# Ruyi-Zha/r2_gaussian

Hardware: AMD Instinct MI355X
Metric: rasterized X-ray views/sec (fwd+bwd) at 300k Gaussians, 512^2 cone-beam detector (higher is better)
Workload: dtype f32

## Files before the change

### r2_gaussian_amd/csrc/raster_geom.hip

```cpp
#include "r2_math.hpp"
#include "raster_state.hpp"

R2_TS_DEFINE(geom)

#ifndef M_PI
#define M_PI 3.14159265358979323846
#endif

namespace r2 {

__device__ __forceinline__ float ndc2pix(float v, int S) { return (float)((((double)v + 1.0) * (double)S - 1.0) * 0.5); }

struct Cov2D {
    float tx, ty, tz;
    float xmul, ymul;
    M3 J, W, M, cov;
};

__device__ __forceinline__ void cov2d_common(float3 mean, float fx, float fy, float tan_fovx, float tan_fovy,
                                             const float *cov3D, const float *__restrict__ view, int mode, Cov2D &c)
{
    float3 t = xform4x3(mean, view);
    if (mode == 0) {
        const float limx = 1.3f, limy = 1.3f;
        t.x = fminf(limx, fmaxf(-limx, t.x));
        t.y = fminf(limx, fmaxf(-limx, t.y));
        c.xmul = (t.x < -limx || t.x > limx) ? 0.f : 1.f;
        c.ymul = (t.y < -limy || t.y > limy) ? 0.f : 1.f;
        c.J = m3(fx, 0.0f, 0.0f, 0.0f, fy, 0.0f, 0.0f, 0.0f, 1.0f);
    } else {
        const float limx = 1.3f * tan_fovx, limy = 1.3f * tan_fovy;
        const float txtz = t.x / t.z, tytz = t.y / t.z;
        t.x = fminf(limx, fmaxf(-limx, txtz)) * t.z;
        t.y = fminf(limy, fmaxf(-limy, tytz)) * t.z;
        c.xmul = (txtz < -limx || txtz > limx) ? 0.f : 1.f;
        c.ymul = (tytz < -limy || tytz > limy) ? 0.f : 1.f;
        const float l = sqrtf(t.x * t.x + t.y * t.y + t.z * t.z);
        c.J = m3(fx / t.z, 0.0f, -(fx * t.x) / (t.z * t.z), 0.0f, fy / t.z, -(fy * t.y) / (t.z * t.z), t.x / l, t.y / l,
                 t.z / l);
    }
    c.tx = t.x; c.ty = t.y; c.tz = t.z;
    c.W = m3(view[0], view[4], view[8], view[1], view[5], view[9], view[2], view[6], view[10]);
    c.M = mul(c.W, c.J);
    const M3 Vrk = m3(cov3D[0], cov3D[1], cov3D[2], cov3D[1], cov3D[3], cov3D[4], cov3D[2], cov3D[4], cov3D[5]);
    c.cov = mul(mul(tr(c.M), tr(Vrk)), c.M);
}

__device__ __forceinline__ float mu_of(float circ, float diamond)
{
    const double q = 2 * M_PI * (double)circ / (double)diamond;
    float mu = 0.0f;
    if ((float)q > 0.0f) mu = (float)sqrt(q);
    return mu;
}

__device__ __forceinline__ void raster_preprocess_one(
    int idx , int src , const float *__restrict__ means3D, const float *__restrict__ scales, float scale_modifier,
    const float *__restrict__ rotations, const float *__restrict__ opacities, const float *__restrict__ cov3D_precomp,
    const float *__restrict__ view, const float *__restrict__ proj, int W, int H, float tan_fovx, float tan_fovy,
    float focal_x, float focal_y, int mode, int gx, int gy,
    int *__restrict__ radii, float4 *__restrict__ rec, uint32_t *__restrict__ depth_key,
    float *__restrict__ cov3Ds, uint32_t *__restrict__ tiles_touched, float2 *__restrict__ op_mu,
    uint32_t *__restrict__ thin_flag, const DepthReg &reg, uint32_t &key_out, uint2 &bt_out, uint32_t &rect_out)
{
    key_out = DEPTH_CULLED_KEY;
    radii[idx] = 0;
    tiles_touched[idx] = 0;
    depth_key[idx] = 0xFFFFFFFFu;

    const float3 p = make_float3(means3D[3 * src], means3D[3 * src + 1], means3D[3 * src + 2]);
    const float3 p_view = xform4x3(p, view);
    if (p_view.z <= 0.2f) return;
    const float4 p_hom = xform4x4(p, proj);
    const float p_w = 1.0f / (p_hom.w + 0.0000001f);
    const float projx = p_hom.x * p_w, projy = p_hom.y * p_w;

    float cov3D[6];
    if (cov3D_precomp != nullptr) {
#pragma unroll
        for (int k = 0; k < 6; ++k) cov3D[k] = cov3D_precomp[6 * src + k];
    } else {
        const float4 q = reinterpret_cast<const float4 *>(rotations)[src];
        cov3d_from_scale_rot(scales[3 * src], scales[3 * src + 1], scales[3 * src + 2], scale_modifier, q, cov3D);
        if (cov3Ds != nullptr)
#pragma unroll
            for (int k = 0; k < 6; ++k) cov3Ds[6 * idx + k] = cov3D[k];
    }

    Cov2D c;
    cov2d_common(p, focal_x, focal_y, tan_fovx, tan_fovy, cov3D, view, mode, c);
    const float a = c.cov.m[0][0], b = c.cov.m[0][1], cc = c.cov.m[0][2];
    const float d = c.cov.m[1][1], e = c.cov.m[1][2], f = c.cov.m[2][2];
    const float diamond = a * d - b * b;
    const float circ = a * d * f + 2 * b * cc * e - a * e * e - f * b * b - d * cc * cc;
    const float mu = mu_of(circ, diamond);

    const float det = (a * d - b * b);
    if (det == 0.0f) return;
    const float det_inv = 1.f / det;
    const float conA = d * det_inv, conB = -b * det_inv, conC = a * det_inv;

    const float mid = 0.5f * (a + d);
    const float lambda1 = mid + sqrtf(fmaxf(0.1f, mid * mid - det));
    const float lambda2 = mid - sqrtf(fmaxf(0.1f, mid * mid - det));
    const float my_radius = ceilf(3.f * sqrtf(fmaxf(lambda1, lambda2)));
    const float px = ndc2pix(projx, W), py = ndc2pix(projy, H);
    int x0, y0, x1, y1;
    tile_rect(px, py, (int)my_radius, gx, gy, x0, y0, x1, y1);
    if ((uint32_t)(x1 - x0) * (uint32_t)(y1 - y0) == 0) return;

    depth_key[idx] = __float_as_uint(p_view.z);
    radii[idx] = (int)my_radius;
    tiles_touched[idx] = (uint32_t)(y1 - y0) * (uint32_t)(x1 - x0);
    key_out = __float_as_uint(p_view.z);
    bt_out = depth_register_key(reg, key_out, (uint32_t)(y1 - y0) * (uint32_t)(x1 - x0));
    rect_out = depth_rect_pack(x0, y0, x1 - x0, y1 - y0);
    const float op = opacities[src];
    const float opmu = op * mu;
    const float L = opmu > 0.0f ? log2f(opmu) : -INFINITY;
    float hx = INFINITY, hy = INFINITY;
    {
        const double qmax = 2.0 * (double)LN2 * ((double)L - (double)LOG2_ALPHA_MIN_2D) + 1e-3;
        const double A = conA, B = conB, C = conC;
        const double det2 = A * C - B * B, trc = A + C;
        if (!(qmax > 0.0)) {
            hx = hy = -INFINITY;
        } else if (det2 > 0.0 && A > 0.0 && C > 0.0 && trc * trc <= 1.0e4 * det2) {
            const double ex = sqrt(qmax * C / det2) * 1.004 + 0.05, ey = sqrt(qmax * A / det2) * 1.004 + 0.05;
            if (ex < 1.0e30 && ey < 1.0e30) { hx = (float)ex; hy = (float)ey; }
        }
    }
    rec[2 * idx] = make_float4(px, py, (-0.5f * LOG2E) * conA, (-LOG2E) * conB);
    rec[2 * idx + 1] = make_float4((-0.5f * LOG2E) * conC, L, hx, hy);
    op_mu[idx] = make_float2(op, mu);
    if (thin_flag && hx > 0.f && item_tier((-0.5f * LOG2E) * conA, (-LOG2E) * conB, (-0.5f * LOG2E) * conC, L, hx, hy) != 0) *thin_flag = 1u;
}

__global__ void __launch_bounds__(256) raster_preprocess_kernel(
    int P, int V, const float *__restrict__ means3D, const float *__restrict__ scales, float scale_modifier,
    const float *__restrict__ rotations, const float *__restrict__ opacities, const float *__restrict__ cov3D_precomp,
    const float *__restrict__ views, const float *__restrict__ projs, int W, int H, float tan_fovx, float tan_fovy,
    float focal_x, float focal_y, int mode, int gx, int gy,
    int *__restrict__ radii, float4 *__restrict__ rec, uint32_t *__restrict__ depth_key,
    float *__restrict__ cov3Ds, uint32_t *__restrict__ tiles_touched, float2 *__restrict__ op_mu,
    uint32_t *__restrict__ thin_flag, DepthReg reg)
{
    const int idx = blockIdx.x * 256 + threadIdx.x;
    R2_TS_AT(geom, 0);
    uint32_t key = DEPTH_CULLED_KEY;
    uint2 bt = make_uint2(0u, 0u);
    uint32_t rect = 0u, thin = 0u;
    if (idx < P * V) {
        const int v = V == 1 ? 0 : idx / P;
        raster_preprocess_one(idx, idx - v * P, means3D, scales, scale_modifier, rotations, opacities, cov3D_precomp, views + 16 * v,
                              projs + 16 * v, W, H, tan_fovx, tan_fovy, focal_x, focal_y, mode, gx, gy, radii, rec, depth_key, cov3Ds,
                              tiles_touched, op_mu, &thin, reg, key, bt, rect);
    }
    if (thin_flag != nullptr) {
        const uint32_t nthin = (uint32_t)__popcll(__ballot(thin != 0u));
        if (nthin != 0u && (threadIdx.x & 63) == 0) atomicAdd(thin_flag, nthin);
    }
    R2_TS_AT(geom, 1);
    depth_register_end(reg, (uint32_t)idx, key, bt, rect);
    R2_TS_AT(geom, 2);
}

template <bool SL , bool SHARE, bool MV>
__global__ void __launch_bounds__(TF_THREADS_MAX, SHARE ? 8 : 4) raster_preprocess_tf_kernel(
    int P , int V ,
    uint32_t per_wg, const TFSlabs slabs, const float *__restrict__ means3D, const float *__restrict__ scales, float scale_modifier,
    const float *__restrict__ rotations, const float *__restrict__ opacities, const float *__restrict__ cov3D_precomp,
    const float *__restrict__ view, const float *__restrict__ proj, int W, int H, float tan_fovx, float tan_fovy,
    float focal_x, float focal_y, int mode, int gx, int gy,
    int *__restrict__ radii, float4 *__restrict__ rec, uint32_t *__restrict__ depth_key,
    float *__restrict__ cov3Ds, uint32_t *__restrict__ tiles_touched, float2 *__restrict__ op_mu,
    uint32_t *__restrict__ first, uint32_t *__restrict__ rects, uint32_t *__restrict__ wgoff, uint32_t *__restrict__ wgmm,
    TFCounters *__restrict__ ctr)
{
    extern __shared__ uint32_t tf_hist[];
    constexpr int MAXW = (int)(TF_THREADS_MAX / 64), NI = (int)TF_PER_THREAD_MAX;
    __shared__ uint32_t s_wn[NI][MAXW], s_wv[MAXW], s_kmx[MAXW], s_nkmn[MAXW], s_thin, s_base;
    const int tid = threadIdx.x, lane = tid & 63, wave = tid >> 6;
    const uint32_t NT = blockDim.x;
    const int nw = (int)(NT >> 6);
    const uint32_t nsl = SL ? slabs.n : 1u;
    const uint32_t T = (uint32_t)(gx * gy * (MV ? V : 1)) * nsl;
    const uint32_t PV = (uint32_t)P * (uint32_t)(MV ? V : 1);
    const uint32_t g0 = blockIdx.x * per_wg, g1 = min(g0 + per_wg, PV);
    R2_TS_AT(geom, 0);
    for (uint32_t t = tid; t < T; t += NT) tf_hist[t] = 0u;
    if (tid == 0) s_thin = 0u;
    uint32_t key[NI], rect[NI], thin = 0u;
    const DepthReg noreg{};
#pragma unroll
    for (int it = 0; it < NI; ++it) {
        key[it] = DEPTH_CULLED_KEY; rect[it] = 0u;
        const uint32_t idx = g0 + (uint32_t)it * NT + (uint32_t)tid;
        uint2 bt = make_uint2(0u, 0u);
        if ((it == 0 || NT * (uint32_t)it < per_wg) && idx < g1) {
            const uint32_t v = MV ? idx / (uint32_t)P : 0u;
            raster_preprocess_one((int)idx, (int)(idx - v * (uint32_t)P), means3D, scales, scale_modifier, rotations, opacities,
                                  cov3D_precomp, view + 16u * v, proj + 16u * v, W, H, tan_fovx, tan_fovy, focal_x, focal_y, mode, gx, gy,
                                  radii, rec, depth_key, cov3Ds, tiles_touched, op_mu, &thin, noreg, key[it], bt, rect[it]);
            if (MV && key[it] != DEPTH_CULLED_KEY) rect[it] += (v * (uint32_t)gy) << 8;
        }
    }
    R2_TS_AT(geom, 10);
    __syncthreads();
    uint32_t n[NI], incl[NI], nvis = 0u, kmx = 0u, nkmn = 0u;
#pragma unroll
    for (int it = 0; it < NI; ++it) {
        const bool vis = key[it] != DEPTH_CULLED_KEY;
        n[it] = vis ? depth_rect_count(rect[it]) : 0u;
        if (vis) {
            const uint32_t x0 = rect[it] & 0xFFu, y0 = (rect[it] >> 8) & 0xFFu, w = ((rect[it] >> 16) & 0xFFu) + 1u, h = (rect[it] >> 24) + 1u;
            const uint32_t sl = SL ? tf_slab_of(key[it], slabs) : 0u;
            for (uint32_t r = 0; r < h; ++r) {
                const uint32_t row = ((y0 + r) * (uint32_t)gx + x0) * nsl + sl;
                for (uint32_t c = 0; c < w; ++c) atomicAdd(&tf_hist[row + c * nsl], 1u);
            }
            rects[g0 + (uint32_t)it * NT + (uint32_t)tid] = rect[it];
            kmx = max(kmx, key[it]);
            nkmn = max(nkmn, ~key[it]);
        }
        incl[it] = n[it];
#pragma unroll
        for (int d = 1; d < 64; d <<= 1) {
            const uint32_t up = __shfl_up(incl[it], d);
            if (lane >= d) incl[it] += up;
        }
        nvis += (uint32_t)__popcll(__ballot(vis));
        if (lane == 63) s_wn[it][wave] = incl[it];
    }
#pragma unroll
    for (int d = 32; d >= 1; d >>= 1) {
        kmx = max(kmx, (uint32_t)__shfl_xor(kmx, d));
        nkmn = max(nkmn, (uint32_t)__shfl_xor(nkmn, d));
    }
    if (lane == 63) { s_wv[wave] = nvis; s_kmx[wave] = kmx; s_nkmn[wave] = nkmn; }
    {
        const uint32_t nthin = (uint32_t)__popcll(__ballot(thin != 0u));
        if (nthin != 0u && lane == 0) atomicAdd(&s_thin, nthin);
    }
    R2_TS_AT(geom, 11);
    __syncthreads();
    R2_TS_AT(geom, 12);
    uint32_t before[NI], tn = 0, tv = 0;
#pragma unroll
    for (int it = 0; it < NI; ++it) {
        before[it] = tn;
        for (int q = 0; q < nw; ++q) {
            if (q < wave) before[it] += s_wn[it][q];
            tn += s_wn[it][q];
        }
    }
    for (int q = 0; q < nw; ++q) tv += s_wv[q];
    unsigned long long base_old = 0ull;
    if (tid == 0) {
        base_old = atomicAdd(&ctr->total, ((unsigned long long)tv << 40) | (unsigned long long)tn);
        if (s_thin) atomicAdd(&ctr->thin, s_thin);
        uint32_t a = 0u, b = 0u;
        for (int q = 0; q < nw; ++q) { a = max(a, s_kmx[q]); b = max(b, s_nkmn[q]); }
        wgmm[2u * blockIdx.x] = a;
        wgmm[2u * blockIdx.x + 1u] = b;
    }
    uint32_t *__restrict__ my_off = wgoff + (size_t)blockIdx.x * T;
    for (uint32_t t = tid; t < T; t += NT) {
        const uint32_t c = tf_hist[t];
        if (c) my_off[t] = atomicAdd(&ctr->tile_count[t], c);
    }
    R2_TS_AT(geom, 13);
    if (tid == 0) s_base = (uint32_t)base_old;
    __syncthreads();
#pragma unroll
    for (int it = 0; it < NI; ++it)
        if (key[it] != DEPTH_CULLED_KEY) first[g0 + (uint32_t)it * NT + (uint32_t)tid] = s_base + before[it] + incl[it] - n[it];
    R2_TS_AT(geom, 1);
}

__global__ void __launch_bounds__(256) mark_visible_kernel(int P, const float *__restrict__ means3D,
                                                           const float *__restrict__ view, uint8_t *__restrict__ present)
{
    const int idx = blockIdx.x * 256 + threadIdx.x;
    if (idx >= P) return;
    const float3 p = make_float3(means3D[3 * idx], means3D[3 * idx + 1], means3D[3 * idx + 2]);
    present[idx] = xform4x3(p, view).z <= 0.2f ? 0 : 1;
}

__global__ void __launch_bounds__(256) raster_duplicate_kernel(
    int P , int Pview, const float4 *__restrict__ rec, const uint32_t *__restrict__ order, const uint32_t *__restrict__ offsets,
    const int *__restrict__ radii, int gx, int gy, uint32_t *__restrict__ first, uint32_t *__restrict__ tiles,
    uint32_t *__restrict__ vals, const uint32_t *__restrict__ nvis)
{
    R2_TS_AT(geom, 4);
    const bool multi_view = Pview != P;
    if (nvis) P = min(P, (int)*nvis);
    const int j = blockIdx.x * 256 + threadIdx.x;
    const int lane = threadIdx.x & 63;
    const int wave_first = j - lane;
    if (wave_first >= P) return;
    uint32_t id = 0;
    int rad = 0;
    if (j < P) {
        id = order[j];
        rad = radii[id];
    }
    const bool live = rad > 0;
    uint32_t excl = 0, incl = 0;
    if (j < P) {
        incl = offsets[j];
        excl = j == 0 ? 0u : offsets[j - 1];
    } else {
        incl = excl = offsets[P - 1];
    }
    int x0 = 0, y0 = 0, x1 = 0, y1 = 0;
    if (live) {
        const float4 r0 = rec[2 * id];
        tile_rect(r0.x, r0.y, rad, gx, gy, x0, y0, x1, y1);
        first[id] = excl;
    }
    const uint32_t wbeg = __shfl(excl, 0);
// ... 486 lines not shown
```

### r2_gaussian_amd/csrc/raster_state.hpp

```cpp
#pragma once
#include "r2_common.hpp"

namespace r2 {

constexpr uint32_t FWD_CHUNK = 1024;
constexpr int PART_STRIDE = 8;
constexpr float ALPHA_MIN_2D = 0.00001f;
constexpr float LOG2_ALPHA_MIN_2D = -16.609640474436812f;
constexpr int SUB2D = 8;

__device__ __forceinline__ void tile_rect(float px, float py, int rad, int gx, int gy, int &x0, int &y0, int &x1, int &y1)
{
    x0 = min(gx, max(0, (int)((px - rad) / TILE2D)));
    y0 = min(gy, max(0, (int)((py - rad) / TILE2D)));
    x1 = min(gx, max(0, (int)((px + rad + TILE2D - 1) / TILE2D)));
    y1 = min(gy, max(0, (int)((py + rad + TILE2D - 1) / TILE2D)));
}

template <bool MV>
__device__ __forceinline__ void tile_decode(uint32_t tile, int gx, int gy, int &tx, int &ty, int &v)
{
    tx = (int)(tile % (uint32_t)gx);
    const int tyt = (int)(tile / (uint32_t)gx);
    v = MV ? tyt / gy : 0;
    ty = tyt - v * gy;
}

__device__ __forceinline__ int row_tier(float A2, float L, float hx)
{
    const float room = __builtin_amdgcn_sqrtf(fmaxf(125.5f + fminf(L, 0.f), 0.f)) - __builtin_amdgcn_sqrtf(fmaxf(L - LOG2_ALPHA_MIN_2D, 0.f) + 1.0f);
    const float s8 = room * (1.0f / 7.0f), s4 = room * (1.0f / 3.0f);
    const float a = fabsf(A2);
    if (!(hx < 3.0e38f) || !(room > 0.f)) return 2;
    return a <= s8 * s8 ? 0 : (a <= s4 * s4 ? 1 : 2);
}
__device__ __forceinline__ bool needs_exact_row(float A2, float L, float hx) { return row_tier(A2, L, hx) == 2; }
__device__ __forceinline__ int item_tier(float A2, float B2, float C2, float L, float hx, float hy)
{
    const float room = __builtin_amdgcn_sqrtf(fmaxf(125.5f + fminf(L, 0.f), 0.f)) - __builtin_amdgcn_sqrtf(fmaxf(L - LOG2_ALPHA_MIN_2D, 0.f) + 1.0f);
    if (!(hx < 3.0e38f) || !(hy < 3.0e38f) || !(room > 0.f)) return 2;
    const float reach2 = 49.0f * fabsf(A2) + 9.0f * fabsf(C2) + 21.0f * fabsf(B2);
    return reach2 <= room * room ? 0 : 2;
}

__device__ __forceinline__ bool block_live(float px, float py, float hx, float hy, float x0, float y0, float n)
{
    return (px - hx <= x0 + (n - 1.0f)) && (px + hx >= x0) && (py - hy <= y0 + (n - 1.0f)) && (py + hy >= y0);
}

__device__ __forceinline__ uint32_t block_mask4(float px, float py, float hx, float hy, int tx, int ty)
{
    const float x0 = (float)(tx * TILE2D), y0 = (float)(ty * TILE2D);
    uint32_t m = 0u;
#pragma unroll
    for (int q = 0; q < 4; ++q)
        if (block_live(px, py, hx, hy, x0 + (float)((q & 1) * SUB2D), y0 + (float)((q >> 1) * SUB2D), (float)SUB2D)) m |= 1u << q;
    return m;
}
constexpr int MASK_BITS = 4;
__device__ __forceinline__ uint32_t ballot_rank(unsigned long long m)
{
    return __builtin_amdgcn_mbcnt_hi((uint32_t)(m >> 32), __builtin_amdgcn_mbcnt_lo((uint32_t)m, 0u));
}


constexpr uint32_t TF_THREADS_MAX = 1024, TF_PER_THREAD_MAX = 2, TF_PER_WG_MIN = 256;
constexpr uint32_t TF_MAX_SLABS = 4;
constexpr uint32_t TF_SLAB_SPLIT_ABOVE = 12288;
struct TFSlabs { uint32_t n, lo; float scale; };
__host__ __device__ __forceinline__ uint32_t tf_slab_of(uint32_t key, const TFSlabs &sl)
{
    const uint32_t k = key > sl.lo ? key - sl.lo : 0u;
    const uint32_t v = (uint32_t)((float)k * sl.scale);
    return v < sl.n - 1u ? v : sl.n - 1u;
}
struct TFGrid { uint32_t wgs, per_wg, threads; };
inline TFGrid tf_grid(int P, int cus)
{
    const unsigned long long cap = (unsigned long long)TF_THREADS_MAX * TF_PER_THREAD_MAX, c = (unsigned long long)(cus > 0 ? cus : 1);
    const unsigned long long k = ((unsigned long long)P + c * cap - 1) / (c * cap);
    unsigned long long per = ((unsigned long long)P + k * c - 1) / (k * c);
    if (per < TF_PER_WG_MIN) per = TF_PER_WG_MIN;
    if (k > 1) per = TF_THREADS_MAX;
    TFGrid g;
    g.per_wg = (uint32_t)per;
    g.wgs = (uint32_t)(((unsigned long long)P + per - 1) / per);
    const unsigned long long th = (per + 63) / 64 * 64;
    g.threads = (uint32_t)(th > TF_THREADS_MAX ? TF_THREADS_MAX : th);
    return g;
}
struct RasterGeom {
    float4 *rec;
    float2 *op_mu;
    uint32_t *depth_key;
    uint32_t *iota;
    uint32_t *depth_sorted;
    uint32_t *order;
    uint32_t *first;
    float *cov3D;
    uint32_t *tiles_touched;
    uint32_t *host_words;
    uint32_t *offsets;
    char *scan_temp;
    size_t scan_bytes;
    char *dorder_temp;
    size_t dorder_bytes;
    char *psort_temp;
    size_t psort_bytes;
    uint32_t *tf_rect;
    uint32_t *tf_wgoff;
    uint32_t *tf_wgmm;
    size_t bytes;
    static RasterGeom carve(char *chunk, int P, size_t tf_T = 0, size_t tf_wgs = 0)
    {
        RasterGeom g;
        Bump b(chunk);
        g.rec = b.take<float4>(2 * (size_t)P);
        g.op_mu = b.take<float2>(P);
        g.depth_key = b.take<uint32_t>(P);
        g.iota = b.take<uint32_t>(P);
        g.depth_sorted = b.take<uint32_t>(P);
        g.order = b.take<uint32_t>(P);
        g.first = b.take<uint32_t>(P);
        g.cov3D = b.take<float>(6 * (size_t)P);
        g.tiles_touched = b.take<uint32_t>(P);
        g.offsets = b.take<uint32_t>(P);
            g.scan_bytes = scan_gather_temp_bytes(P);
        g.scan_temp = b.take<char>(g.scan_bytes);
        g.dorder_bytes = depth_order_temp_bytes((size_t)P);
        g.dorder_temp = b.take<char>(g.dorder_bytes);
        g.host_words = chunk ? depth_order_words(g.dorder_temp, (size_t)P) : nullptr;
        g.psort_bytes = sort_temp_bytes((size_t)P);
        g.psort_temp = b.take<char>(g.psort_bytes);
        g.tf_rect = b.take<uint32_t>(tf_T ? (size_t)P : 0);
        g.tf_wgoff = b.take<uint32_t>(tf_wgs * tf_T);
        g.tf_wgmm = b.take<uint32_t>(tf_wgs * 2);
        g.bytes = b.total();
        return g;
    }
};

struct RasterBinning {
    uint32_t *tiles_unsorted;
    uint32_t *tiles;
    uint32_t *masked;
    uint32_t *vals_unsorted;
    uint32_t *inv;
    uint32_t *point_list;
    float *part;
    char *sort_temp;
    size_t sort_bytes;
    size_t bytes;
    static RasterBinning carve(char *chunk, size_t R)
    {
        RasterBinning s;
        Bump b(chunk);
        s.point_list = b.take<uint32_t>(R);
        s.tiles = b.take<uint32_t>(R);
        s.masked = b.take<uint32_t>(R);
        s.tiles_unsorted = b.take<uint32_t>(R);
        s.vals_unsorted = b.take<uint32_t>(R);
        s.inv = b.take<uint32_t>(R);
        s.part = b.take<float>(R * PART_STRIDE);
        s.sort_bytes = sort_temp_bytes(R);
        s.sort_temp = b.take<char>(s.sort_bytes);
        s.bytes = b.total();
        return s;
    }
};

__host__ __device__ __forceinline__ uint32_t *binning_tiles_ptr(char *base, size_t R)
{
    return reinterpret_cast<uint32_t *>(base + (((R * sizeof(uint32_t)) + 127) & ~size_t(127)));
}
__host__ __device__ __forceinline__ uint32_t *binning_masked_ptr(char *base, size_t R)
{
    return reinterpret_cast<uint32_t *>(base + 2 * (((R * sizeof(uint32_t)) + 127) & ~size_t(127)));
}

constexpr uint32_t TF_SMALL_CAP = 1536;
constexpr uint32_t TF_MAX_TILES = 4096;
constexpr int TF_NOT_TAKEN = -1000001;
constexpr uint32_t TF_MARK = 0x71FEu;
struct TFCounters {
    unsigned long long total;
    uint32_t unused;
    uint32_t thin;
    uint32_t pad[12];
    uint32_t tile_count[TF_MAX_TILES];
};

struct RasterImage {
    uint2 *ranges;
    uint32_t *chunk_base;
    uint32_t *tile_done;
    uint4 *work_tile;
    float *partial;
    uint32_t *partial_last;
    uint32_t *n_contrib;
    char *work_temp;
    uint4 *tf_parts;
    size_t NP;
    size_t NW;
    size_t bytes;
    static RasterImage carve(char *chunk, size_t T, size_t N, size_t R, bool debug, size_t tf_lists = 0)
    {
        RasterImage s;
        Bump b(chunk);
        s.NW = R / FWD_CHUNK + T;
        s.ranges = b.take<uint2>(T);
        s.chunk_base = b.take<uint32_t>(T + 2);
        s.tile_done = b.take<uint32_t>(4 * T);
        s.work_tile = b.take<uint4>(s.NW);
        s.partial = b.take<float>(s.NW * 256);
        s.partial_last = b.take<uint32_t>(debug ? s.NW * 256 : 0);
        s.n_contrib = b.take<uint32_t>(debug ? N : 0);
        s.work_temp = b.take<char>(build_work_temp_bytes(T));
// ... 52 lines not shown
```

### r2_gaussian_amd/csrc/raster_tilefirst.hip

```cpp
#include "raster_state.hpp"
#include "dispatch.hpp"

#include <algorithm>
#include <atomic>
#include <cstdlib>
#include <vector>

R2_TS_DEFINE(tilefirst)

namespace r2 {

namespace {

constexpr int TFS_THREADS = (int)TF_THREADS_MAX;
constexpr int TFK_THREADS = 1024;
constexpr int TFK_GROUPS = TFK_THREADS / 256;
constexpr uint32_t TFK_SMALL_CAP = 1536, TFK_SMALL_PER = 6, TFK_SMALL_BINS = 1024;
constexpr uint32_t TFK_BIG_CAP = 8192, TFK_BIG_PER = 8, TFK_BIG_BINS = 2048;
constexpr uint32_t TFK_BIG_TARGET = 5120;
constexpr uint32_t TFK_COARSE = 1024;
constexpr size_t TFK_LDS = TFK_BIG_CAP * sizeof(unsigned long long) + (TFK_BIG_BINS + 1 + TFK_COARSE + 1) * sizeof(uint32_t);
static_assert(TFK_GROUPS * TFK_SMALL_CAP * sizeof(unsigned long long) + TFK_GROUPS * (TFK_SMALL_BINS + 1) * sizeof(uint32_t) <= TFK_LDS,
              "the groups fit the big layout");
static_assert(TFK_SMALL_CAP == TF_SMALL_CAP && TFK_COARSE == TFK_THREADS && TFK_BIG_CAP >= TFK_BIG_TARGET + TFK_BIG_TARGET / 2,
              "parts need slack over their target size");

constexpr uint32_t TFS_SERVICE = 3;
template <bool SL >
__global__ void __launch_bounds__(TFS_THREADS) raster_tf_scatter_kernel(
    int P , int Pv , int gy, uint32_t per_wg, uint32_t pthreads, int gx,
    uint32_t T , const TFSlabs slabs,
    const uint32_t *__restrict__ rects, const float4 *__restrict__ rec,
    const uint32_t *__restrict__ depth_key, const uint32_t *__restrict__ tiles_touched, const uint32_t *__restrict__ wgoff,
    const uint32_t *__restrict__ wgmm, uint32_t producers, const TFCounters *__restrict__ ctr, uint32_t *__restrict__ words,
    uint32_t *__restrict__ mailbox, uint32_t seq, uint32_t cap, uint2 *__restrict__ pairs, WorkListOut wo,
    uint4 *__restrict__ big_parts, uint32_t big_cap, uint4 *__restrict__ small_tiles,
    uint32_t *__restrict__ nparts )
{
    extern __shared__ uint32_t s_pos[];
    __shared__ uint32_t s_wsum[3][TFS_THREADS / 64], s_carry[3];
    const int tid = threadIdx.x, lane = tid & 63, wave = tid >> 6;
    const uint32_t *__restrict__ tile_count = ctr->tile_count;
    R2_TS_AT(tilefirst, 0);
    const unsigned long long tot = ctr->total;
    const uint32_t R = tf_total_instances(tot);
    if (blockIdx.x == 0) {
        uint32_t gkmax = 0u, gnkmin = 0u;
        for (uint32_t b = tid; b < producers; b += TFS_THREADS) {
            gkmax = max(gkmax, wgmm[2u * b]);
            gnkmin = max(gnkmin, wgmm[2u * b + 1u]);
        }
#pragma unroll
        for (int d = 32; d >= 1; d >>= 1) {
            gkmax = max(gkmax, (uint32_t)__shfl_xor(gkmax, d));
            gnkmin = max(gnkmin, (uint32_t)__shfl_xor(gnkmin, d));
        }
        if (lane == 0) { s_wsum[0][wave] = gkmax; s_wsum[1][wave] = gnkmin; }
        __syncthreads();
        if (tid == 0) {
#pragma unroll
            for (int q = 0; q < TFS_THREADS / 64; ++q) { gkmax = max(gkmax, s_wsum[0][q]); gnkmin = max(gnkmin, s_wsum[1][q]); }
            const uint32_t nvis = (uint32_t)(tot >> 40), any_thin = ctr->thin;
            words[DW_TOTAL] = R; words[DW_OVERFLOW] = 0u; words[DW_USER] = any_thin; words[DW_PMAX] = TF_MARK;
            words[DW_PNMAX] = 0u; words[DW_NMAX] = gkmax; words[DW_NNMAX] = gnkmin; words[DW_NVIS] = nvis;
            if (mailbox != nullptr) {
                mailbox[DW_TOTAL] = R; mailbox[DW_OVERFLOW] = 0u; mailbox[DW_USER] = any_thin; mailbox[DW_PMAX] = TF_MARK;
                mailbox[DW_PNMAX] = 0u; mailbox[DW_NMAX] = gkmax; mailbox[DW_NNMAX] = gnkmin; mailbox[DW_NVIS] = nvis;
                __hip_atomic_store(&mailbox[15], seq, __ATOMIC_RELEASE, __HIP_MEMORY_SCOPE_SYSTEM);
            }
        }
        __syncthreads();
        R2_TS_AT(tilefirst, 5);
    }
    if (R > cap) {
        if (blockIdx.x == 0 && tid == 0) { wo.chunk_base[wo.T] = 0u; wo.chunk_base[wo.T + 1] = 0u; nparts[0] = 0u; nparts[1] = 0u; }
        return;
    }
    if (blockIdx.x == 0) return;
    if (blockIdx.x == 1) {
        if (SL) {
            for (uint32_t t = tid; t < wo.T; t += TFS_THREADS) {
                uint32_t c = 0u;
                for (uint32_t d = 0; d < slabs.n; ++d) c += tile_count[t * slabs.n + d];
                s_pos[t] = c;
            }
            __syncthreads();
        }
        ranges_and_work_block<TFS_THREADS>(SL ? s_pos : tile_count, wo);
        R2_TS_AT(tilefirst, 2);
        return;
    }
    if (blockIdx.x == 2) {
        if (tid < 3) s_carry[tid] = 0u;
        __syncthreads();
        for (uint32_t base = 0; base < T; base += TFS_THREADS) {
            const uint32_t t = base + (uint32_t)tid;
            const uint32_t c = t < T ? tile_count[t] : 0u;
            const uint32_t nb = c > TFK_SMALL_CAP ? (c > TFK_BIG_CAP ? (c + TFK_BIG_TARGET - 1u) / TFK_BIG_TARGET : 1u) : 0u;
            const uint32_t ns = (c != 0u && nb == 0u) ? 1u : 0u;
            uint32_t i0 = c, i1 = nb, i2 = ns;
#pragma unroll
            for (int d = 1; d < 64; d <<= 1) {
                const uint32_t u0 = __shfl_up(i0, d), u1 = __shfl_up(i1, d), u2 = __shfl_up(i2, d);
                if (lane >= d) { i0 += u0; i1 += u1; i2 += u2; }
            }
            if (lane == 63) { s_wsum[0][wave] = i0; s_wsum[1][wave] = i1; s_wsum[2][wave] = i2; }
            __syncthreads();
            uint32_t o0 = 0, o1 = 0, o2 = 0;
            for (int w = 0; w < wave; ++w) { o0 += s_wsum[0][w]; o1 += s_wsum[1][w]; o2 += s_wsum[2][w]; }
            const uint32_t start = s_carry[0] + o0 + i0 - c, bstart = s_carry[1] + o1 + i1 - nb, sstart = s_carry[2] + o2 + i2 - ns;
            for (uint32_t q = 0; q < nb; ++q)
                if (bstart + q < big_cap) big_parts[bstart + q] = make_uint4(t, q | (nb << 16), start, c);
            if (ns) small_tiles[sstart] = make_uint4(t, 0u, start, c);
            __syncthreads();
            if (tid == TFS_THREADS - 1) { s_carry[0] = start + c; s_carry[1] = bstart + nb; s_carry[2] = sstart + ns; }
            __syncthreads();
        }
        if (tid == 0) { nparts[0] = min(s_carry[1], big_cap); nparts[1] = s_carry[2]; }
        R2_TS_AT(tilefirst, 2);
        return;
    }
    const uint32_t wg = blockIdx.x - TFS_SERVICE;
    constexpr int NI = (int)TF_PER_THREAD_MAX;
    const uint32_t g0 = wg * per_wg, g1 = min(g0 + per_wg, (uint32_t)P);
    uint32_t g_idx[NI], g_tt[NI], g_rect[NI], g_key[NI];
    float4 g_box[NI];
#pragma unroll
    for (int it = 0; it < NI; ++it) {
        g_idx[it] = g0 + (uint32_t)it * pthreads + (uint32_t)tid;
        const bool own = (uint32_t)tid < pthreads && g_idx[it] < g1;
        const uint32_t idc = min(g_idx[it], (uint32_t)P - 1u);
        g_tt[it] = tiles_touched[idc]; g_rect[it] = rects[idc]; g_key[it] = depth_key[idc];
        const float4 ra = rec[2u * idc], rb = rec[2u * idc + 1u];
        g_box[it] = make_float4(ra.x, ra.y, rb.z, rb.w);
        g_tt[it] = own ? g_tt[it] : 0u;
    }
    const uint32_t *__restrict__ my_off = wgoff + (size_t)wg * T;
    constexpr int MAXT = (int)(TF_MAX_TILES / TFS_THREADS);
    uint32_t offs[MAXT];
#pragma unroll
    for (int q = 0; q < MAXT; ++q) {
        const uint32_t t = (uint32_t)(q * TFS_THREADS + tid);
        offs[q] = my_off[min(t, T - 1u)];
        s_pos[min(t, T - 1u)] = tile_count[min(t, T - 1u)];
    }
    __syncthreads();
    const uint32_t ipt = (T + TFS_THREADS - 1) / TFS_THREADS;
    const uint32_t t0 = (uint32_t)tid * ipt, t1 = min(t0 + ipt, T);
    uint32_t sum = 0;
    for (uint32_t t = t0; t < t1; ++t) sum += s_pos[t];
    uint32_t incl = sum;
#pragma unroll
    for (int d = 1; d < 64; d <<= 1) {
        const uint32_t up = __shfl_up(incl, d);
        if (lane >= d) incl += up;
    }
    if (lane == 63) s_wsum[0][wave] = incl;
    __syncthreads();
    uint32_t run = incl - sum;
    for (int w = 0; w < wave; ++w) run += s_wsum[0][w];
    for (uint32_t t = t0; t < t1; ++t) {
        const uint32_t c = s_pos[t];
        s_pos[t] = run;
        run += c;
    }
    __syncthreads();
#pragma unroll
    for (int q = 0; q < MAXT; ++q) {
        const uint32_t t = (uint32_t)(q * TFS_THREADS + tid);
        if (t < T) s_pos[t] += offs[q];
    }
    __syncthreads();
#pragma unroll
    for (int it = 0; it < NI; ++it)
        if (g_tt[it] != 0u) {
            const uint32_t rect = g_rect[it], key = g_key[it];
            const uint32_t x0 = rect & 0xFFu, y0 = (rect >> 8) & 0xFFu, w = ((rect >> 16) & 0xFFu) + 1u, h = (rect >> 24) + 1u;
            const uint32_t nsl = SL ? slabs.n : 1u, sl = SL ? tf_slab_of(key, slabs) : 0u;
            const uint32_t idw = g_idx[it] << MASK_BITS;
            const uint32_t yoff = Pv == P ? 0u : (g_idx[it] / (uint32_t)Pv) * (uint32_t)gy;
            const float lim = 1048576.0f;
            const int Ax = (int)fminf(fmaxf(ceilf(g_box[it].x - g_box[it].z), -lim), lim);
            const int Bx = (int)fminf(fmaxf(floorf(g_box[it].x + g_box[it].z), -lim), lim);
            const int Ay = (int)fminf(fmaxf(ceilf(g_box[it].y - g_box[it].w), -lim), lim);
            const int By = (int)fminf(fmaxf(floorf(g_box[it].y + g_box[it].w), -lim), lim);
            auto axis_mask = [](int A, int B, int origin) -> uint32_t {
                const int lo = max((A - origin) >> 3, 0), hi = min((B - origin) >> 3, 31);
                return lo > hi ? 0u : ((0xFFFFFFFFu >> (31 - hi)) & (0xFFFFFFFFu << lo));
            };
            const int X0 = (int)(x0 * (uint32_t)TILE2D), Y0 = (int)((y0 - yoff) * (uint32_t)TILE2D);
            const uint32_t xm0 = axis_mask(Ax, Bx, X0);
            uint32_t ym = 0u;
            for (uint32_t r = 0; r < h; ++r) {
                const uint32_t row = ((y0 + r) * (uint32_t)gx + x0) * nsl + sl;
                if ((r & 15u) == 0u) ym = axis_mask(Ay, By, Y0 + (int)(r * (uint32_t)TILE2D));
                const uint32_t yb = (ym >> (2u * (r & 15u))) & 3u;
                const uint32_t ymul = (yb & 1u) | ((yb & 2u) << 1);
                for (uint32_t c0 = 0; c0 < w; c0 += 16u) {
                    const uint32_t xm = c0 == 0u ? xm0 : axis_mask(Ax, Bx, X0 + (int)(c0 * (uint32_t)TILE2D));
                    const uint32_t c1 = min(w, c0 + 16u);
                    for (uint32_t c = c0; c < c1; ++c) {
                        const uint32_t xb = (xm >> (2u * (c - c0))) & 3u;
                        const uint32_t pos = atomicAdd(&s_pos[row + c * nsl], 1u);
                        pairs[pos] = make_uint2(key, idw | (xb * ymul));
                    }
                }
            }
        }
    R2_TS_AT(tilefirst, 1);
}

__device__ __forceinline__ unsigned long long tf_pack(const uint2 e) { return ((unsigned long long)e.x << 32) | (unsigned long long)e.y; }

template <int NT>
__device__ __forceinline__ void tf_group_minmax(uint32_t &kmin, uint32_t &kmax, uint32_t (*s_mm)[TFK_THREADS / 64], int lane, int wave, int w0)
{
#pragma unroll
    for (int d = 32; d >= 1; d >>= 1) {
        kmin = min(kmin, (uint32_t)__shfl_xor(kmin, d));
        kmax = max(kmax, (uint32_t)__shfl_xor(kmax, d));
    }
    __syncthreads();
    if (lane == 0) { s_mm[0][wave] = kmin; s_mm[1][wave] = kmax; }
    __syncthreads();
#pragma unroll
    for (int w = 0; w < NT / 64; ++w) { kmin = min(kmin, s_mm[0][w0 + w]); kmax = max(kmax, s_mm[1][w0 + w]); }
}

template <int NT, uint32_t PER, uint32_t BINS>
__device__ __forceinline__ void tf_sort_group(unsigned long long (&mine)[PER], unsigned long long *s_a, uint32_t *s_bin,
                                              uint32_t *s_wsum , int gtid, int lane, int wave, int w0,
                                              uint32_t cnt, uint32_t kmin, uint32_t kmax, uint32_t *__restrict__ dst,
                                              uint32_t *__restrict__ dst_masked)
{
    R2_TS_AT(tilefirst, 6);
    for (uint32_t i = gtid; i <= BINS; i += NT) s_bin[i] = 0u;
    __syncthreads();
    const float scale = kmax > kmin ? (float)(BINS - 1) / (float)(kmax - kmin) : 0.f;
    uint32_t my_bin[PER], my_ticket[PER];
#pragma unroll
    for (uint32_t u = 0; u < PER; ++u) {
        const uint32_t i = u * NT + (uint32_t)gtid;
        my_bin[u] = 0u; my_ticket[u] = 0u;
        if (i < cnt) {
            my_bin[u] = min((uint32_t)((float)((uint32_t)(mine[u] >> 32) - kmin) * scale), BINS - 1u);
            my_ticket[u] = atomicAdd(&s_bin[my_bin[u]], 1u);
        }
    }
    __syncthreads();
    R2_TS_AT(tilefirst, 7);
    {
        constexpr uint32_t BPT = BINS / NT;
        static_assert(BINS % NT == 0, "whole buckets per thread");
        uint32_t c[BPT], tsum = 0;
#pragma unroll
        for (uint32_t q = 0; q < BPT; ++q) { c[q] = s_bin[gtid * BPT + q]; tsum += c[q]; }
        uint32_t incl = tsum;
#pragma unroll
        for (int d = 1; d < 64; d <<= 1) {
            const uint32_t up = __shfl_up(incl, d);
            if (lane >= d) incl += up;
        }
        if (lane == 63) s_wsum[wave] = incl;
        __syncthreads();
        uint32_t run = incl - tsum;
        for (int w = w0; w < wave; ++w) run += s_wsum[w];
#pragma unroll
        for (uint32_t q = 0; q < BPT; ++q) { s_bin[gtid * BPT + q] = run; run += c[q]; }
// ... 412 lines not shown
    uint32_t rmax = 0, kmax = 0, kmin = 0;
    if (const TFHint *hint = tf_hint(P, V, width, height, false); hint && hint->n != 0u) {
        for (uint32_t i = 0; i < std::min(hint->n, 8u); ++i) rmax = std::max(rmax, hint->recent[i]);
        kmax = hint->kmax; kmin = hint->kmin;
    } else if (const TFHint *near = tf_hint_nearby(V, width, height)) {
        uint32_t r0 = 0;
        for (uint32_t i = 0; i < std::min(near->n, 8u); ++i) r0 = std::max(r0, near->recent[i]);
        const double f = (double)P / (double)near->P;
        rmax = (uint32_t)std::min<double>((double)r0 * f * 1.1, 2.0e9);
        kmax = near->kmax; kmin = near->kmin;
        g_tf_seeded.fetch_add(1, std::memory_order_relaxed);
        path_count(PS_RAS_EVENT_SEEDED);
    } else {
        path_count(PS_RAS_GENERAL_NO_PREDICTION);
        g_tf_declined.fetch_add(1, std::memory_order_relaxed);
        return TF_NOT_TAKEN;
    }
    int dev = 0;
    R2_HIP_TRY(hipGetDevice(&dev));
    TFWorkspace *ws = tf_workspace(dev, s);
    if (!ws) {
        path_count(PS_RAS_GENERAL_NO_WORKSPACE);
        g_tf_declined.fetch_add(1, std::memory_order_relaxed);
        return TF_NOT_TAKEN;
    }
    path_count(PS_RAS_TILE_FIRST);
    const bool defer = defer_enabled();
    size_t cap = (((size_t)rmax + (defer ? rmax / 2 : rmax / 4) + 16384) + 65535) & ~(size_t)65535;

    TFSlabs slabs{1u, kmin, 0.f};
    {
        const double ml = 8.0 * (double)rmax / (double)T;
        uint32_t d = 1u;
        if (ml > (double)TF_SLAB_SPLIT_ABOVE)
            while (d < TF_MAX_SLABS && T * d * 2u <= TF_MAX_TILES) d *= 2u;
        if (kmax <= kmin) d = 1u;
        slabs.n = d;
        slabs.scale = d > 1u ? (float)d / ((float)(kmax - kmin) + 1.0f) : 0.f;
        if (d > 1u) path_count(PS_RAS_EVENT_DEPTH_SLABS);
    }
    const size_t TL = T * slabs.n;

    char *gchunk = geometryBuffer(RasterGeom::carve(nullptr, PV, TL, wgs).bytes, geometry_user);
    if (!gchunk) {
        set_error("%s: state allocation callback returned NULL", what);
        return R2_ERR_ALLOC;
    }
    const RasterGeom geom = RasterGeom::carve(gchunk, PV, TL, wgs);
    if (ws->dirty)
        R2_HIP_TRY(hipMemsetAsync(ws->ctr, 0, sizeof(TFCounters) + 64, s));
    ws->dirty = true;
    uint32_t *mailbox = nullptr, mailbox_seq = 0;
    int rc = 0, token = -1;
    if (defer && cap < (size_t)DEFER_TOKEN_FLAG) {
        token = defer_acquire(&mailbox, &mailbox_seq, (uint32_t)cap);
        if (token < 0) g_defer_no_slot.fetch_add(1, std::memory_order_relaxed);
    }
    if (token < 0) rc = host_mailbox_arm(&mailbox, &mailbox_seq);
    if (rc) return rc;
    { StageScope t(ST_RAS_PREPROCESS, s);
    launch_raster_preprocess_tf(geom, P, V, grid, slabs, means3D, scales, scale_modifier, rotations, opacities, cov3D_precomp, viewmatrix,
                                projmatrix, width, height, tan_fovx, tan_fovy, mode, radii, ws->ctr, s); }
    R2_HIP_TRY(hipGetLastError());

    RasterBinning bin{};
    RasterImage img{};
    bool post_mailbox = true;
    auto enqueue = [&](size_t capacity, bool render_only) -> int {
        if (!render_only) {
            char *bchunk = binningBuffer(RasterBinning::carve(nullptr, capacity).bytes, binning_user);
            char *ichunk = imageBuffer(RasterImage::carve(nullptr, T, N, capacity, false, TL).bytes, image_user);
            if (!bchunk || !ichunk) {
                set_error("%s: binning/image allocation callback returned NULL", what);
                return R2_ERR_ALLOC;
            }
            bin = RasterBinning::carve(bchunk, capacity);
            img = RasterImage::carve(ichunk, T, N, capacity, false, TL);
            uint2 *pairs = reinterpret_cast<uint2 *>(bin.part);
            { StageScope t(ST_RAS_DUPLICATE, s);
            const WorkListOut wo{img.ranges, img.chunk_base, img.work_tile, (uint32_t)T, FWD_CHUNK, img.tile_done, 0u, (uint32_t)img.NW,
                                 1u };
#define R2_TF_SCATTER(SLB)                                                                                                        \
            raster_tf_scatter_kernel<SLB><<<dim3((unsigned)wgs + TFS_SERVICE), dim3(TFS_THREADS), TL * sizeof(uint32_t), s>>>(         \
                PV, P, gy, grid.per_wg, grid.threads, gx, (uint32_t)TL, slabs, geom.tf_rect, geom.rec, geom.depth_key, geom.tiles_touched, geom.tf_wgoff, \
                geom.tf_wgmm, (uint32_t)wgs, ws->ctr, geom.host_words, post_mailbox ? mailbox : nullptr, mailbox_seq,                   \
                (uint32_t)std::min<size_t>(capacity, 0x7FFFFFFFu), pairs, wo, img.tf_parts, (uint32_t)img.NP, img.tf_parts + img.NP,   \
                ws->nparts)
            if (slabs.n > 1u) R2_TF_SCATTER(true);
            else R2_TF_SCATTER(false);
#undef R2_TF_SCATTER
            }
            R2_HIP_TRY(hipGetLastError());
            { StageScope t(ST_RAS_SORT, s);
            raster_tf_sort_kernel<<<dim3((unsigned)(img.NP + (TL + TFK_GROUPS - 1) / TFK_GROUPS)), dim3(TFK_THREADS), TFK_LDS, s>>>(
                img.tf_parts, (uint32_t)img.NP, img.tf_parts + img.NP, ws->nparts, pairs, bin.point_list, ws->ctr, geom.host_words,
                (uint32_t)std::min<size_t>(capacity, 0x7FFFFFFFu), token >= 0 ? (uint32_t)TL : 0u); }
            R2_HIP_TRY(hipGetLastError());
        } else {
            R2_HIP_TRY(hipMemsetAsync(img.tile_done, 0, 4 * T * sizeof(uint32_t), s));
        }
        { StageScope t(ST_RAS_RENDER_FWD, s);
        launch_raster_render_forward(geom, bin, img, width, height, V, out_color, false, bin.tiles, true, s,
                                     reinterpret_cast<char *>(bin.point_list), geom.host_words, (size_t)PV); }
        R2_HIP_TRY(hipGetLastError());
        return 0;
    };
    rc = enqueue(cap, false);
    if (rc) return rc;
    if (token >= 0) {
        ws->dirty = false;
        g_tf_taken.fetch_add(1, std::memory_order_relaxed);
        g_defer_taken.fetch_add(1, std::memory_order_relaxed);
        path_count(PS_RAS_EVENT_DEFERRED);
        g_tf_pending.push_back(TFPending{token, P, V, width, height});
        host_mark_wait_begin();
        host_mark_wait_end();
        return token;
    }
    uint32_t hw[DW_COUNT] = { 0 };
    rc = host_mailbox_wait(mailbox_seq, hw, DW_COUNT, s);
    if (rc) return rc;
    const uint32_t num_rendered = hw[DW_TOTAL];
    const bool thin = hw[DW_USER] != 0u;
    if (num_rendered > 0x7FFFFFFFu) {
        set_error("%s: more than 2147483647 (tile, Gaussian) instances: they do not fit the 31-bit num_rendered", what);
        return R2_ERR_INVALID;
    }
    post_mailbox = false;
    if ((size_t)num_rendered > cap) {
        g_tf_rerun.fetch_add(1, std::memory_order_relaxed);
        path_count(PS_RAS_EVENT_SECOND_PASS);
        rc = enqueue(num_rendered, false);
        if (rc) return rc;
    }
    ws->dirty = false;
    g_tf_taken.fetch_add(1, std::memory_order_relaxed);
    raster_tilefirst_note(P, V, width, height, num_rendered, thin, hw[DW_NMAX], ~hw[DW_NNMAX]);
    return (int)num_rendered;
}

void raster_tilefirst_release() { g_tf_ws.release(); g_tf_hints.clear(); g_tf_pending.clear(); }

int raster_resolve_deferred(const char *what, int token, hipStream_t s, uint32_t *num_rendered, bool release)
{
    uint32_t hw[DW_COUNT] = { 0 }, cap = 0;
    const int rc = defer_resolve(token, hw, DW_COUNT, &cap, s, release);
    if (rc) return rc;
    if (defer_count_short(token, hw[DW_TOTAL], cap)) {
        set_error("%s: the deferred forward's state was sized for %u instances, the scene has %u: its image and state are invalid "
                  "(R2_DEFER_COUNT / r2_defer_count_control trade the exact second pass for the missing wait; render this view again "
                  "with the mode off)", what, cap, hw[DW_TOTAL]);
        return R2_ERR_INVALID;
    }
    *num_rendered = hw[DW_TOTAL];
    return 0;
}

}

extern "C" void r2_tile_first_stats(long long *out, int reset)
{
    std::atomic<long long> *c[5] = {&r2::g_tf_taken, &r2::g_tf_declined, &r2::g_tf_rerun, &r2::g_tf_rerender, &r2::g_tf_seeded};
    for (int i = 0; i < 5; ++i) {
        if (out) out[i] = c[i]->load(std::memory_order_relaxed);
        if (reset) c[i]->store(0, std::memory_order_relaxed);
    }
}
// ... 34 lines not shown
```

Before: 6207.

## Pack per-Gaussian handoff into one uint4 and use DPP wave scans

The preprocess kernel now writes a single uint4 per Gaussian holding the rect, depth key and pixel bounds packed as 16-bit pairs. The scatter kernel then does one coalesced load instead of gathering tiles_touched, rects, depth_key and two float4 rec entries, and it no longer recomputes bounds. Shuffle-based wave scans and reductions are replaced with DPP row operations. The packing clamps bounds to the int16 range, which changes the earlier clamp of ±1048576. The DPP scan pattern also needs to be correct for 64-lane waves.

```diff
diff --git a/r2_gaussian_amd/csrc/raster_geom.hip b/r2_gaussian_amd/csrc/raster_geom.hip
--- a/r2_gaussian_amd/csrc/raster_geom.hip
+++ b/r2_gaussian_amd/csrc/raster_geom.hip
@@ -61,9 +61,11 @@
     float focal_x, float focal_y, int mode, int gx, int gy,
     int *__restrict__ radii, float4 *__restrict__ rec, uint32_t *__restrict__ depth_key,
     float *__restrict__ cov3Ds, uint32_t *__restrict__ tiles_touched, float2 *__restrict__ op_mu,
-    uint32_t *__restrict__ thin_flag, const DepthReg &reg, uint32_t &key_out, uint2 &bt_out, uint32_t &rect_out)
+    uint32_t *__restrict__ thin_flag, const DepthReg &reg, uint32_t &key_out, uint2 &bt_out, uint32_t &rect_out,
+    uint2 &bounds_out )
 {
     key_out = DEPTH_CULLED_KEY;
+    bounds_out = make_uint2(0u, 0u);
     radii[idx] = 0;
     tiles_touched[idx] = 0;
     depth_key[idx] = 0xFFFFFFFFu;
@@ -130,6 +132,7 @@
             if (ex < 1.0e30 && ey < 1.0e30) { hx = (float)ex; hy = (float)ey; }
         }
     }
+    bounds_out = make_uint2(tf_pack_bounds(px, hx), tf_pack_bounds(py, hy));
     rec[2 * idx] = make_float4(px, py, (-0.5f * LOG2E) * conA, (-LOG2E) * conB);
     rec[2 * idx + 1] = make_float4((-0.5f * LOG2E) * conC, L, hx, hy);
     op_mu[idx] = make_float2(op, mu);
@@ -150,11 +153,12 @@
     uint32_t key = DEPTH_CULLED_KEY;
     uint2 bt = make_uint2(0u, 0u);
     uint32_t rect = 0u, thin = 0u;
+    uint2 bounds;
     if (idx < P * V) {
         const int v = V == 1 ? 0 : idx / P;
         raster_preprocess_one(idx, idx - v * P, means3D, scales, scale_modifier, rotations, opacities, cov3D_precomp, views + 16 * v,
                               projs + 16 * v, W, H, tan_fovx, tan_fovy, focal_x, focal_y, mode, gx, gy, radii, rec, depth_key, cov3Ds,
-                              tiles_touched, op_mu, &thin, reg, key, bt, rect);
+                              tiles_touched, op_mu, &thin, reg, key, bt, rect, bounds);
     }
     if (thin_flag != nullptr) {
         const uint32_t nthin = (uint32_t)__popcll(__ballot(thin != 0u));
@@ -174,7 +178,7 @@
     float focal_x, float focal_y, int mode, int gx, int gy,
     int *__restrict__ radii, float4 *__restrict__ rec, uint32_t *__restrict__ depth_key,
     float *__restrict__ cov3Ds, uint32_t *__restrict__ tiles_touched, float2 *__restrict__ op_mu,
-    uint32_t *__restrict__ first, uint32_t *__restrict__ rects, uint32_t *__restrict__ wgoff, uint32_t *__restrict__ wgmm,
+    uint32_t *__restrict__ first, uint4 *__restrict__ handoff , uint32_t *__restrict__ wgoff, uint32_t *__restrict__ wgmm,
     TFCounters *__restrict__ ctr)
 {
     extern __shared__ uint32_t tf_hist[];
@@ -196,13 +200,14 @@
     for (int it = 0; it < NI; ++it) {
         key[it] = DEPTH_CULLED_KEY; rect[it] = 0u;
         const uint32_t idx = g0 + (uint32_t)it * NT + (uint32_t)tid;
-        uint2 bt = make_uint2(0u, 0u);
+        uint2 bt = make_uint2(0u, 0u), bounds;
         if ((it == 0 || NT * (uint32_t)it < per_wg) && idx < g1) {
             const uint32_t v = MV ? idx / (uint32_t)P : 0u;
             raster_preprocess_one((int)idx, (int)(idx - v * (uint32_t)P), means3D, scales, scale_modifier, rotations, opacities,
                                   cov3D_precomp, view + 16u * v, proj + 16u * v, W, H, tan_fovx, tan_fovy, focal_x, focal_y, mode, gx, gy,
-                                  radii, rec, depth_key, cov3Ds, tiles_touched, op_mu, &thin, noreg, key[it], bt, rect[it]);
+                                  radii, rec, depth_key, cov3Ds, tiles_touched, op_mu, &thin, noreg, key[it], bt, rect[it], bounds);
             if (MV && key[it] != DEPTH_CULLED_KEY) rect[it] += (v * (uint32_t)gy) << 8;
+            handoff[idx] = make_uint4(rect[it], key[it], bounds.x, bounds.y);
         }
     }
     R2_TS_AT(geom, 10);
@@ -219,24 +224,15 @@
                 const uint32_t row = ((y0 + r) * (uint32_t)gx + x0) * nsl + sl;
                 for (uint32_t c = 0; c < w; ++c) atomicAdd(&tf_hist[row + c * nsl], 1u);
             }
-            rects[g0 + (uint32_t)it * NT + (uint32_t)tid] = rect[it];
             kmx = max(kmx, key[it]);
             nkmn = max(nkmn, ~key[it]);
         }
-        incl[it] = n[it];
-#pragma unroll
-        for (int d = 1; d < 64; d <<= 1) {
-            const uint32_t up = __shfl_up(incl[it], d);
-            if (lane >= d) incl[it] += up;
-        }
+        incl[it] = wave_scan_dpp<false>(n[it]);
         nvis += (uint32_t)__popcll(__ballot(vis));
         if (lane == 63) s_wn[it][wave] = incl[it];
     }
-#pragma unroll
-    for (int d = 32; d >= 1; d >>= 1) {
-        kmx = max(kmx, (uint32_t)__shfl_xor(kmx, d));
-        nkmn = max(nkmn, (uint32_t)__shfl_xor(nkmn, d));
-    }
+    kmx = wave_scan_dpp<true>(kmx);
+    nkmn = wave_scan_dpp<true>(nkmn);
     if (lane == 63) { s_wv[wave] = nvis; s_kmx[wave] = kmx; s_nkmn[wave] = nkmn; }
     {
         const uint32_t nthin = (uint32_t)__popcll(__ballot(thin != 0u));
diff --git a/r2_gaussian_amd/csrc/raster_state.hpp b/r2_gaussian_amd/csrc/raster_state.hpp
--- a/r2_gaussian_amd/csrc/raster_state.hpp
+++ b/r2_gaussian_amd/csrc/raster_state.hpp
@@ -58,9 +58,34 @@
     return m;
 }
 constexpr int MASK_BITS = 4;
+__device__ __forceinline__ uint32_t tf_pack_bounds(float p, float h)
+{
+    const int A = (int)fminf(fmaxf(ceilf(p - h), -32768.0f), 32767.0f), B = (int)fminf(fmaxf(floorf(p + h), -32768.0f), 32767.0f);
+    return ((uint32_t)A & 0xFFFFu) | ((uint32_t)B << 16);
+}
+__device__ __forceinline__ int tf_bound_lo(uint32_t w) { return (int)(w << 16) >> 16; }
+__device__ __forceinline__ int tf_bound_hi(uint32_t w) { return (int)w >> 16; }
 __device__ __forceinline__ uint32_t ballot_rank(unsigned long long m)
 {
     return __builtin_amdgcn_mbcnt_hi((uint32_t)(m >> 32), __builtin_amdgcn_mbcnt_lo((uint32_t)m, 0u));
+}
+
+template <bool MAX>
+__device__ __forceinline__ uint32_t wave_scan_dpp(uint32_t v)
+{
+#define R2_DPP_STEP(ctrl, rows)                                                                                         \
+    {                                                                                                                   \
+        const uint32_t t = (uint32_t)__builtin_amdgcn_update_dpp(0, (int)v, ctrl, rows, 0xF, false);                    \
+        v = MAX ? max(v, t) : v + t;                                                                                    \
+    }
+    R2_DPP_STEP(0x111, 0xF)
+    R2_DPP_STEP(0x112, 0xF)
+    R2_DPP_STEP(0x114, 0xF)
+    R2_DPP_STEP(0x118, 0xF)
+    R2_DPP_STEP(0x142, 0xA)
+    R2_DPP_STEP(0x143, 0xC)
+#undef R2_DPP_STEP
+    return v;
 }
 
 
@@ -107,7 +132,7 @@
     size_t dorder_bytes;
     char *psort_temp;
     size_t psort_bytes;
-    uint32_t *tf_rect;
+    uint4 *tf_rect;
     uint32_t *tf_wgoff;
     uint32_t *tf_wgmm;
     size_t bytes;
@@ -132,7 +157,7 @@
         g.host_words = chunk ? depth_order_words(g.dorder_temp, (size_t)P) : nullptr;
         g.psort_bytes = sort_temp_bytes((size_t)P);
         g.psort_temp = b.take<char>(g.psort_bytes);
-        g.tf_rect = b.take<uint32_t>(tf_T ? (size_t)P : 0);
+        g.tf_rect = b.take<uint4>(tf_T ? (size_t)P : 0);
         g.tf_wgoff = b.take<uint32_t>(tf_wgs * tf_T);
         g.tf_wgmm = b.take<uint32_t>(tf_wgs * 2);
         g.bytes = b.total();
diff --git a/r2_gaussian_amd/csrc/raster_tilefirst.hip b/r2_gaussian_amd/csrc/raster_tilefirst.hip
--- a/r2_gaussian_amd/csrc/raster_tilefirst.hip
+++ b/r2_gaussian_amd/csrc/raster_tilefirst.hip
@@ -30,8 +30,8 @@
 __global__ void __launch_bounds__(TFS_THREADS) raster_tf_scatter_kernel(
     int P , int Pv , int gy, uint32_t per_wg, uint32_t pthreads, int gx,
     uint32_t T , const TFSlabs slabs,
-    const uint32_t *__restrict__ rects, const float4 *__restrict__ rec,
-    const uint32_t *__restrict__ depth_key, const uint32_t *__restrict__ tiles_touched, const uint32_t *__restrict__ wgoff,
+    const uint4 *__restrict__ handoff ,
+    const uint32_t *__restrict__ wgoff,
     const uint32_t *__restrict__ wgmm, uint32_t producers, const TFCounters *__restrict__ ctr, uint32_t *__restrict__ words,
     uint32_t *__restrict__ mailbox, uint32_t seq, uint32_t cap, uint2 *__restrict__ pairs, WorkListOut wo,
     uint4 *__restrict__ big_parts, uint32_t big_cap, uint4 *__restrict__ small_tiles,
@@ -123,17 +123,15 @@
     const uint32_t wg = blockIdx.x - TFS_SERVICE;
     constexpr int NI = (int)TF_PER_THREAD_MAX;
     const uint32_t g0 = wg * per_wg, g1 = min(g0 + per_wg, (uint32_t)P);
-    uint32_t g_idx[NI], g_tt[NI], g_rect[NI], g_key[NI];
-    float4 g_box[NI];
+    uint32_t g_idx[NI];
+    uint4 g_rec[NI];
+    bool g_vis[NI];
 #pragma unroll
     for (int it = 0; it < NI; ++it) {
         g_idx[it] = g0 + (uint32_t)it * pthreads + (uint32_t)tid;
         const bool own = (uint32_t)tid < pthreads && g_idx[it] < g1;
-        const uint32_t idc = min(g_idx[it], (uint32_t)P - 1u);
-        g_tt[it] = tiles_touched[idc]; g_rect[it] = rects[idc]; g_key[it] = depth_key[idc];
-        const float4 ra = rec[2u * idc], rb = rec[2u * idc + 1u];
-        g_box[it] = make_float4(ra.x, ra.y, rb.z, rb.w);
-        g_tt[it] = own ? g_tt[it] : 0u;
+        g_rec[it] = handoff[min(g_idx[it], (uint32_t)P - 1u)];
+        g_vis[it] = own && g_rec[it].y != DEPTH_CULLED_KEY;
     }
     const uint32_t *__restrict__ my_off = wgoff + (size_t)wg * T;
     constexpr int MAXT = (int)(TF_MAX_TILES / TFS_THREADS);
@@ -149,12 +147,7 @@
     const uint32_t t0 = (uint32_t)tid * ipt, t1 = min(t0 + ipt, T);
     uint32_t sum = 0;
     for (uint32_t t = t0; t < t1; ++t) sum += s_pos[t];
-    uint32_t incl = sum;
-#pragma unroll
-    for (int d = 1; d < 64; d <<= 1) {
-        const uint32_t up = __shfl_up(incl, d);
-        if (lane >= d) incl += up;
-    }
+    const uint32_t incl = wave_scan_dpp<false>(sum);
     if (lane == 63) s_wsum[0][wave] = incl;
     __syncthreads();
     uint32_t run = incl - sum;
@@ -171,19 +164,17 @@
         if (t < T) s_pos[t] += offs[q];
     }
     __syncthreads();
+    R2_TS_AT(tilefirst, 10);
 #pragma unroll
     for (int it = 0; it < NI; ++it)
-        if (g_tt[it] != 0u) {
-            const uint32_t rect = g_rect[it], key = g_key[it];
+        if (g_vis[it]) {
+            const uint32_t rect = g_rec[it].x, key = g_rec[it].y;
             const uint32_t x0 = rect & 0xFFu, y0 = (rect >> 8) & 0xFFu, w = ((rect >> 16) & 0xFFu) + 1u, h = (rect >> 24) + 1u;
             const uint32_t nsl = SL ? slabs.n : 1u, sl = SL ? tf_slab_of(key, slabs) : 0u;
             const uint32_t idw = g_idx[it] << MASK_BITS;
             const uint32_t yoff = Pv == P ? 0u : (g_idx[it] / (uint32_t)Pv) * (uint32_t)gy;
-            const float lim = 1048576.0f;
-            const int Ax = (int)fminf(fmaxf(ceilf(g_box[it].x - g_box[it].z), -lim), lim);
-            const int Bx = (int)fminf(fmaxf(floorf(g_box[it].x + g_box[it].z), -lim), lim);
-            const int Ay = (int)fminf(fmaxf(ceilf(g_box[it].y - g_box[it].w), -lim), lim);
-            const int By = (int)fminf(fmaxf(floorf(g_box[it].y + g_box[it].w), -lim), lim);
+            const int Ax = tf_bound_lo(g_rec[it].z), Bx = tf_bound_hi(g_rec[it].z);
+            const int Ay = tf_bound_lo(g_rec[it].w), By = tf_bound_hi(g_rec[it].w);
             auto axis_mask = [](int A, int B, int origin) -> uint32_t {
                 const int lo = max((A - origin) >> 3, 0), hi = min((B - origin) >> 3, 31);
                 return lo > hi ? 0u : ((0xFFFFFFFFu >> (31 - hi)) & (0xFFFFFFFFu << lo));
@@ -762,7 +753,7 @@
                                  1u };
 #define R2_TF_SCATTER(SLB)                                                                                                        \
             raster_tf_scatter_kernel<SLB><<<dim3((unsigned)wgs + TFS_SERVICE), dim3(TFS_THREADS), TL * sizeof(uint32_t), s>>>(         \
-                PV, P, gy, grid.per_wg, grid.threads, gx, (uint32_t)TL, slabs, geom.tf_rect, geom.rec, geom.depth_key, geom.tiles_touched, geom.tf_wgoff, \
+                PV, P, gy, grid.per_wg, grid.threads, gx, (uint32_t)TL, slabs, geom.tf_rect, geom.tf_wgoff,                             \
                 geom.tf_wgmm, (uint32_t)wgs, ws->ctr, geom.host_words, post_mailbox ? mailbox : nullptr, mailbox_seq,                   \
                 (uint32_t)std::min<size_t>(capacity, 0x7FFFFFFFu), pairs, wo, img.tf_parts, (uint32_t)img.NP, img.tf_parts + img.NP,   \
                 ws->nparts)
```

New measurement: 6161 (median of 5 runs). Within noise of the previous version (-0.7%).
